# RainbowZL0/swin-unet-image-fusion

Measured on AMD Instinct MI355X. Metric: fused image-pairs/sec at 256x256, win=8, higher is better.
Workload: dtype bf16; 1 GPU; B=16/GPU 256x256 IR/visible pairs, win=8, 5-level Swin-UNet fusion forward (BASELINE configs[1]); global_batch=16, precision_mode=fast, residual_stream=fp32, hip_graph=True, steps_in_flight=3, kernel_schedule=throughput, collective=none, weights=random-init (numpy PCG64 recipe, seed 0)

## Files before the change

### swin_unet_image_fusion_amd/csrc/kernels_win48.hip

```cpp
#include "kernels_win48.h"
#include "win_frag.h"

#include <algorithm>

namespace swf {
namespace {

using namespace wf;

constexpr int W48_WAVES = 2;

template <int HID_>
struct G48 {
    static constexpr int C = 48, HID = HID_, HEADS = 8, D = 6;
    static constexpr int NT1 = HID / 32, KU = HID / 16;
    static_assert(HID % 32 == 0, "hidden tiles");
    static constexpr int F_QKV = 0;
    static constexpr int F_P = 36;
    static constexpr int F_W1 = 52;
    static constexpr int F_W2 = F_W1 + 6 * NT1;
    static constexpr int NFRAG = F_W2 + 4 * KU;
    static constexpr int V_LN1G = 0, V_LN1B = 24, V_LN2G = 48, V_LN2B = 72, V_B2 = 96, V_BQ = 120, V_BK = 152, V_B1 = 184, VHF = 288;
    static_assert(V_B1 + 16 * NT1 <= VHF, "vector block");
    static constexpr int VSTREAM = 2 * VHF + 64;
    static constexpr size_t p_vec = size_t(NFRAG) * 1024;
    static constexpr size_t p_bias = (p_vec + size_t(VSTREAM) * 4 + 15) / 16 * 16;
    static constexpr size_t p_total = p_bias + size_t(2) * 2 * 16 * 64 * 4;
    static constexpr size_t l_k = 0, l_v = 16 * 1024, l_vec = 32 * 1024, l_total = l_vec + size_t(2) * VSTREAM * 4;
    static constexpr size_t p_total16 = p_bias + size_t(15) * 16 * 64 * 4;
    static constexpr size_t l_k16 = 0, l_v16 = 32 * 1024, l_vec16 = 64 * 1024, l_total16 = l_vec16 + size_t(2) * VSTREAM * 4;
};

struct Win48Args {
    const float* in[2];
    float* out[2];
    const char* packed[2];
    const char* warm[2];
    int B, H, W, shift, cross, warm_bytes;
    int ntok[2];
};

constexpr int W48_BLOCK = 0, W48_ATTN = 1, W48_MLP = 2;

__device__ __forceinline__ void raw48(const f32x16& x0, const f32x16& x1, u32x4 (&xh)[3], u32x4 (&xl)[3]) {
    float n[24];
#pragma unroll
    for (int i = 0; i < 24; ++i) n[i] = i < 16 ? x0[i] : x1[i - 16];
    split8(n, xh[0], xl[0]);
    split8(n + 8, xh[1], xl[1]);
    split8(n + 16, xh[2], xl[2]);
}

__device__ __forceinline__ void layernorm48(const f32x16& x0, const f32x16& x1, const float* vec, int goff, int boff, u32x4 (&xh)[3], u32x4 (&xl)[3]) {
    float s = 0.f;
#pragma unroll
    for (int i = 0; i < 16; ++i) s += x0[i];
#pragma unroll
    for (int i = 0; i < 8; ++i) s += x1[i];
    const float mean = sum_halves(s) * (1.0f / 48.0f);
    float d[24], q = 0.f;
#pragma unroll
    for (int i = 0; i < 24; ++i) {
        d[i] = (i < 16 ? x0[i] : x1[i - 16]) - mean;
        q += d[i] * d[i];
    }
    const float rstd = __builtin_amdgcn_rsqf(sum_halves(q) * (1.0f / 48.0f) + 1e-5f);
    float n[24];
#pragma unroll
    for (int a = 0; a < 6; ++a) {
        const float4 g = *reinterpret_cast<const float4*>(vec + goff + 4 * a);
        const float4 b = *reinterpret_cast<const float4*>(vec + boff + 4 * a);
        n[4 * a + 0] = d[4 * a + 0] * rstd * g.x + b.x;
        n[4 * a + 1] = d[4 * a + 1] * rstd * g.y + b.y;
        n[4 * a + 2] = d[4 * a + 2] * rstd * g.z + b.z;
        n[4 * a + 3] = d[4 * a + 3] * rstd * g.w + b.w;
    }
    split8(n, xh[0], xl[0]);
    split8(n + 8, xh[1], xl[1]);
    split8(n + 16, xh[2], xl[2]);
}

__device__ __forceinline__ void attention48(const u32x4* ksrc, const u32x4* vsrc, const u32x4 (&qf)[2][2], const f32x16 (&bias)[2],
                                            bool half1, f32x16 (&o)[2]) {
    const f32x16 zero16 = {0.f, 0.f, 0.f, 0.f, 0.f, 0.f, 0.f, 0.f, 0.f, 0.f, 0.f, 0.f, 0.f, 0.f, 0.f, 0.f};
    o[0] = zero16;
    o[1] = zero16;
#pragma unroll
    for (int h = 0; h < 8; ++h) {
        const int T = h >> 2, hq = h & 3, sp = hq >> 1, sub = hq & 1;
        const u32x4 ka0 = ksrc[((0 * 2 + T) * 2 + sp) * 64], ka1 = ksrc[((1 * 2 + T) * 2 + sp) * 64];
        u32x4 qm = {0u, 0u, 0u, 0u};
        qm[2 * sub] = qf[T][sp][2 * sub];
        qm[2 * sub + 1] = qf[T][sp][2 * sub + 1];
        float mx;
        {
            f32x16 s0 = mfma_f16(ka0, qm, bias[0]);
            mx = max3f(s0[0], s0[1], s0[2]);
#pragma unroll
            for (int i = 3; i < 15; i += 2) mx = max3f(mx, s0[i], s0[i + 1]);
            mx = __builtin_fmaxf(mx, s0[15]);
        }
        {
            f32x16 s1 = mfma_f16(ka1, qm, bias[1]);
#pragma unroll
            for (int i = 0; i < 16; i += 2) mx = max3f(mx, s1[i], s1[i + 1]);
        }
        mx = max_halves(mx);
        {
            const f16 nm = (f16)(-mx);
            qm[2 * sub + 1] |= half1 ? ((unsigned)__builtin_bit_cast(unsigned short, nm) << 16) : 0u;
        }
        f32x16 t;
#pragma unroll
        for (int kt = 0; kt < 2; ++kt) {
            f32x16 sc = mfma_f16(kt ? ka1 : ka0, qm, bias[kt]);
#pragma unroll
            for (int s2 = 0; s2 < 2; ++s2) {
                float p[8];
#pragma unroll
                for (int j = 0; j < 8; ++j) p[j] = __builtin_amdgcn_exp2f(sc[8 * s2 + j]);
                const u32x4 pf = pack8_f16(p);
                const u32x4 va = vsrc[(T * 4 + 2 * kt + s2) * 64];
                t = mfma_f16(va, pf, (kt == 0 && s2 == 0) ? zero16 : t);
                __builtin_amdgcn_sched_barrier(0);
            }
        }
#pragma unroll
        for (int j = 0; j < 4; ++j) o[T][4 * hq + j] = t[4 * hq + j];
        __builtin_amdgcn_sched_barrier(0);
    }
}

template <int HID, int WS, int MODE = W48_BLOCK, bool RAW = false>
__global__ __launch_bounds__(256, W48_WAVES) void window48_kernel(Win48Args args) {
    using G = G48<HID>;
    static_assert(WS == 7 || WS == 8, "window side");
    static_assert(!RAW || MODE != W48_BLOCK, "RAW belongs to the half-block modes");
    constexpr bool ATT = MODE != W48_MLP, MLP = MODE != W48_ATTN;
    __shared__ __attribute__((aligned(16))) char smem[G::l_total];
    u32x4* kimg = reinterpret_cast<u32x4*>(smem + G::l_k);
    u32x4* vimg = reinterpret_cast<u32x4*>(smem + G::l_v);
    float* lvec = reinterpret_cast<float*>(smem + G::l_vec);

    const int tid = threadIdx.x, lane = tid & 63, wave = tid >> 6;
    const int ws = wave >> 1, qb = wave & 1, r = lane & 31, hf = lane >> 5;
    const int H = args.H, W = args.W, nwx = ATT ? W / WS : 1, nwy = ATT ? H / WS : 1, npi = nwx * nwy;
    const int nwin = ATT ? args.B * npi : (max(args.ntok[0], args.ntok[1]) + 63) / 64;
    const int sh = args.shift ? WS / 2 : 0;
    const int kvs = args.cross ? 1 - ws : ws;

    const __amdgpu_buffer_rsrc_t wrs = __builtin_amdgcn_make_buffer_rsrc(const_cast<char*>(uniform_ptr(args.packed[ws])), 0, (int)G::p_total, 0x00020000);
    const __amdgpu_buffer_rsrc_t krs = __builtin_amdgcn_make_buffer_rsrc(const_cast<char*>(uniform_ptr(args.packed[kvs])), 0, (int)G::p_total, 0x00020000);
    const int act_bytes = ATT ? args.B * H * W * 48 * 4 : args.ntok[ws] * 48 * 4;
    const __amdgpu_buffer_rsrc_t irs = __builtin_amdgcn_make_buffer_rsrc(const_cast<float*>(uniform_ptr(args.in[ws])), 0, act_bytes, 0x00020000);
    const __amdgpu_buffer_rsrc_t ors = __builtin_amdgcn_make_buffer_rsrc(uniform_ptr(args.out[ws]), 0, (MODE == W48_BLOCK || args.out[ws]) ? act_bytes : 0, 0x00020000);
    const unsigned loff = (unsigned)lane * 16u;
    auto WF = [&](int f) { return __builtin_bit_cast(u32x4, __builtin_amdgcn_raw_buffer_load_b128(wrs, loff, f * 1024, 0)); };
    auto WK = [&](int f) { return __builtin_bit_cast(u32x4, __builtin_amdgcn_raw_buffer_load_b128(krs, loff, f * 1024, 0)); };
    const float* vec = lvec + ws * G::VSTREAM + hf * G::VHF;
    const float* veck = lvec + kvs * G::VSTREAM + hf * G::VHF;
    const float* vecv = lvec + kvs * G::VSTREAM + 2 * G::VHF;
    const bool half1 = hf != 0;
    const bool col_masked = half1 != (((r >> 2) & 1) != 0);
    const f32x16 zero16 = {0.f, 0.f, 0.f, 0.f, 0.f, 0.f, 0.f, 0.f, 0.f, 0.f, 0.f, 0.f, 0.f, 0.f, 0.f, 0.f};

    for (int win = blockIdx.x; win < nwin; win += gridDim.x) {
        SWF_WF_FENCE();
        const int b = win / npi, wrem = win - b * npi;
        const int wy = wrem / nwx, wx = wrem - wy * nwx;
        const int ty = 4 * qb + (r >> 3), tx = r & 7;
        int oy = wy * WS + ty + sh, ox = wx * WS + tx + sh;
        oy = oy >= H ? oy - H : oy;
        ox = ox >= W ? ox - W : ox;
        const unsigned tokoff = [&]() -> unsigned {
            if constexpr (ATT) {
                return (WS == 8 || (ty < WS && tx < WS)) ? (unsigned)((((b * H + oy) * W + ox) * 48 + 4 * hf) * 4) : 0x80000000u;
            } else {
                const int tok = 64 * win + 32 * qb + r;
                return tok < args.ntok[ws] ? (unsigned)((tok * 48 + 4 * hf) * 4) : 0x80000000u;
            }
        }();
        auto load_rows = [&](f32x16& t0, f32x16& t1) {
#pragma unroll
            for (int a = 0; a < 6; ++a) {
                const f32x4 v = __builtin_bit_cast(f32x4, __builtin_amdgcn_raw_buffer_load_b128(irs, tokoff, 32 * a, 0));
                if (a < 4) { t0[4 * a] = v.x; t0[4 * a + 1] = v.y; t0[4 * a + 2] = v.z; t0[4 * a + 3] = v.w; }
                else { t1[4 * (a - 4)] = v.x; t1[4 * (a - 4) + 1] = v.y; t1[4 * (a - 4) + 2] = v.z; t1[4 * (a - 4) + 3] = v.w; }
            }
#pragma unroll
            for (int i = 8; i < 16; ++i) t1[i] = 0.f;
        };

        f32x16 res0, res1;
        if constexpr (ATT) {
        u32x4 qf[2][2];
        {
            u32x4 wq[2][6];
            auto req = [&](int ph, u32x4 (&dst)[6]) {
                const int m = ph >> 1, T = ph & 1;
#pragma unroll
                for (int i = 0; i < 6; ++i) dst[i] = m == 0 ? WF(G::F_QKV + ((m * 2 + T) * 3) * 2 + i) : WK(G::F_QKV + ((m * 2 + T) * 3) * 2 + i);
            };
            req(0, wq[0]);
            f32x16 x0, x1;
            load_rows(x0, x1);
            if (win == (int)blockIdx.x) {
                static_assert(G::VSTREAM % 4 == 0 && G::p_vec % 16 == 0, "vector sections move as 16-byte groups");
                    fill_vectors<G::VSTREAM / 4, 256>(lvec, args.packed[0] + G::p_vec, args.packed[1] + G::p_vec, tid);
                __syncthreads();
            }
            u32x4 xh[3], xl[3];
            if constexpr (RAW) raw48(x0, x1, xh, xl);
            else layernorm48(x0, x1, vec, G::V_LN1G, G::V_LN1B, xh, xl);
            float t[16];
#pragma unroll
            for (int ph = 0; ph < 6; ++ph) {
                const int m = ph >> 1, T = ph & 1;
                SWF_WF_FENCE();
                if (ph + 1 < 6) req(ph + 1, wq[(ph + 1) & 1]);
                SWF_WF_FENCE();
                const u32x4 (&w)[6] = wq[ph & 1];
                f32x16 acc = zero16;
                if (RAW && (m == 0 ? ws == 1 : ws == 0)) {
                    if (ph == 2 && win != (int)blockIdx.x) __syncthreads();
                } else if (m < 2) {
#pragma unroll
                    for (int s = 0; s < 3; ++s) acc = mma3(w[2 * s], w[2 * s + 1], xh[s], xl[s], acc);
                    const float* bsrc = m == 0 ? vec + G::V_BQ : veck + G::V_BK;
#pragma unroll
                    for (int g = 0; g < 4; ++g) {
                        const float4 bb = *reinterpret_cast<const float4*>(bsrc + 16 * T + 4 * g);
                        t[4 * g] = acc[4 * g] + bb.x; t[4 * g + 1] = acc[4 * g + 1] + bb.y; t[4 * g + 2] = acc[4 * g + 2] + bb.z; t[4 * g + 3] = acc[4 * g + 3] + bb.w;
                    }
                    if (m == 0) {
                        qf[T][0] = pack8_f16(t);
                        qf[T][1] = pack8_f16(t + 8);
                    } else {
                        if (T == 0 && win != (int)blockIdx.x) __syncthreads();
                        u32x4* kdst = kimg + (((kvs * 2 + qb) * 2 + T) * 2) * 64 + lane;
                        kdst[0] = pack8_f16(t);
                        kdst[64] = pack8_f16(t + 8);
                    }
                } else {
#pragma unroll
                    for (int s = 0; s < 3; ++s) acc = mma3(xh[s], xl[s], w[2 * s], w[2 * s + 1], acc);
                    const float bv = vecv[32 * T + r];
#pragma unroll
                    for (int i = 0; i < 16; ++i) t[i] = acc[i] + bv;
                    u32x4* vdst = vimg + ((kvs * 2 + T) * 4 + 2 * qb) * 64 + lane;
                    vdst[0] = pack8_f16(t);
                    vdst[64] = pack8_f16(t + 8);
                }
            }
        }
        f32x16 bias[2];
#pragma unroll
        for (int kt = 0; kt < 2; ++kt)
#pragma unroll
            for (int a = 0; a < 4; ++a) {
                const f32x4 v = __builtin_bit_cast(f32x4, __builtin_amdgcn_raw_buffer_load_b128(wrs, loff, (int)G::p_bias + ((__builtin_amdgcn_readfirstlane(qb) * 2 + kt) * 4 + a) * 1024, 0));
                bias[kt][4 * a] = v.x; bias[kt][4 * a + 1] = v.y; bias[kt][4 * a + 2] = v.z; bias[kt][4 * a + 3] = v.w;
            }
        __syncthreads();
        if (RAW && ws == 1) continue;

        f32x16 o[2];
        {
            const bool rowv = args.shift && wy == nwy - 1, colv = args.shift && wx == nwx - 1;
            const u32x4* ksrc = kimg + (ws * 8) * 64 + lane;
            const u32x4* vsrc = vimg + (ws * 8) * 64 + lane;
            if (rowv || colv) {
                const float pen0 = ((rowv && qb == 1) || (colv && col_masked)) ? -INFINITY : 0.f;
                const float pen1 = ((rowv && qb == 0) || (colv && col_masked)) ? -INFINITY : 0.f;
#pragma unroll
                for (int i = 0; i < 16; ++i) { bias[0][i] += pen0; bias[1][i] += pen1; }
            }
            attention48(ksrc, vsrc, qf, bias, half1, o);
        }

        u32x4 wpj[16];
        SWF_WF_FENCE();
        if constexpr (RAW) { res0 = zero16; res1 = zero16; }
        else load_rows(res0, res1);
#pragma unroll
        for (int i = 0; i < 16; ++i) wpj[i] = WF(G::F_P + i);
        SWF_WF_FENCE();
        {
            u32x4 oh[4], ol[4];
#pragma unroll
            for (int T = 0; T < 2; ++T) {
                float t[16];
#pragma unroll
                for (int q = 0; q < 4; ++q) {
                    float lo_, den;
                    halves(o[T][4 * q + 2], lo_, den);
                    const float inv = __builtin_amdgcn_rcpf(den);
                    t[4 * q] = o[T][4 * q] * inv; t[4 * q + 1] = o[T][4 * q + 1] * inv; t[4 * q + 2] = o[T][4 * q + 2] * inv; t[4 * q + 3] = o[T][4 * q + 3] * inv;
                }
                split8(t, oh[2 * T], ol[2 * T]);
                split8(t + 8, oh[2 * T + 1], ol[2 * T + 1]);
            }
#pragma unroll
            for (int ks = 0; ks < 4; ++ks) {
                res0 = mma3(wpj[(0 * 4 + ks) * 2], wpj[(0 * 4 + ks) * 2 + 1], oh[ks], ol[ks], res0);
                res1 = mma3(wpj[(1 * 4 + ks) * 2], wpj[(1 * 4 + ks) * 2 + 1], oh[ks], ol[ks], res1);
            }
        }

        } else {
            load_rows(res0, res1);
            if (win == (int)blockIdx.x) {
                fill_vectors<G::VSTREAM / 4, 256>(lvec, args.packed[0] + G::p_vec, args.packed[1] + G::p_vec, tid);
                __syncthreads();
            }
        }

        if constexpr (MLP) {
            u32x4 w1[2][6];
            auto req1 = [&](int tI, u32x4 (&dst)[6]) {
#pragma unroll
                for (int i = 0; i < 6; ++i) dst[i] = WF(G::F_W1 + tI * 6 + i);
            };
            u32x4 w2[2][2][2][2];
            auto req2 = [&](int tI, u32x4 (&dst)[2][2][2]) {
#pragma unroll
                for (int To = 0; To < 2; ++To)
#pragma unroll
                    for (int s2 = 0; s2 < 2; ++s2) {
                        dst[To][s2][0] = WF(G::F_W2 + (To * G::KU + 2 * tI + s2) * 2);
                        dst[To][s2][1] = WF(G::F_W2 + (To * G::KU + 2 * tI + s2) * 2 + 1);
                    }
            };
            req1(0, w1[0]);
            req2(0, w2[0]);
            u32x4 xh[3], xl[3];
            if constexpr (RAW) { raw48(res0, res1, xh, xl); res0 = zero16; res1 = zero16; }
            else layernorm48(res0, res1, vec, G::V_LN2G, G::V_LN2B, xh, xl);
#pragma unroll
            for (int tI = 0; tI < G::NT1; ++tI) {
                SWF_WF_FENCE();
                if (tI + 1 < G::NT1) { req1(tI + 1, w1[(tI + 1) & 1]); req2(tI + 1, w2[(tI + 1) & 1]); }
                SWF_WF_FENCE();
                const u32x4 (&w)[6] = w1[tI & 1];
                f32x16 acc = zero16;
#pragma unroll
                for (int s = 0; s < 3; ++s) acc = mma3(w[2 * s], w[2 * s + 1], xh[s], xl[s], acc);
                float e[16];
#pragma unroll
                for (int g = 0; g < 4; ++g) {
                    const float4 b1 = *reinterpret_cast<const float4*>(vec + G::V_B1 + 16 * tI + 4 * g);
                    const float bb[4] = {b1.x, b1.y, b1.z, b1.w};
#pragma unroll
                    for (int j = 0; j < 4; ++j) {
                        const float u = acc[4 * g + j] + bb[j];
                        const float L = __builtin_fmaf(__builtin_amdgcn_exp2f(u), kLog2e, -kLog2e);
                        e[4 * g + j] = __builtin_amdgcn_fmed3f(u, L, 0.f);
                    }
                }
#pragma unroll
                for (int s2 = 0; s2 < 2; ++s2) {
                    u32x4 hh, hl;
                    split8(e + 8 * s2, hh, hl);
                    res0 = mma3(w2[tI & 1][0][s2][0], w2[tI & 1][0][s2][1], hh, hl, res0);
                    res1 = mma3(w2[tI & 1][1][s2][0], w2[tI & 1][1][s2][1], hh, hl, res1);
                }
                __builtin_amdgcn_sched_barrier(0);
            }
#pragma unroll
            for (int a = 0; a < 6; ++a) {
                const float4 b2 = *reinterpret_cast<const float4*>(vec + G::V_B2 + 4 * a);
                if (a < 4) { res0[4 * a] += b2.x; res0[4 * a + 1] += b2.y; res0[4 * a + 2] += b2.z; res0[4 * a + 3] += b2.w; }
                else { res1[4 * (a - 4)] += b2.x; res1[4 * (a - 4) + 1] += b2.y; res1[4 * (a - 4) + 2] += b2.z; res1[4 * (a - 4) + 3] += b2.w; }
            }
        }

#pragma unroll
        for (int a = 0; a < 6; ++a) {
            const f32x4 v = a < 4 ? f32x4{res0[4 * a], res0[4 * a + 1], res0[4 * a + 2], res0[4 * a + 3]}
                                  : f32x4{res1[4 * (a - 4)], res1[4 * (a - 4) + 1], res1[4 * (a - 4) + 2], res1[4 * (a - 4) + 3]};
            __builtin_amdgcn_raw_buffer_store_b128(__builtin_bit_cast(u32x4, v), ors, tokoff, 32 * a, 0);
        }
    }

    if (args.warm[0]) {
        const int nsl = max(1, (int)gridDim.x / 8), sl = ((int)blockIdx.x / 8) % nsl;
        const int lines = (args.warm_bytes + 127) / 128;
        const int per = (lines + nsl - 1) / nsl, l0 = sl * per, l1 = min(lines, l0 + per);
        unsigned acc = 0;
        for (int s2 = 0; s2 < 2; ++s2)
            for (int l = l0 + tid; l < l1; l += 256) acc ^= *reinterpret_cast<const unsigned*>(args.warm[s2] + (size_t)l * 128);
        if (acc == 0x9e3779b9u && args.B < 0) args.out[0][0] = 0.f;
    }
}

template <int HID>
__global__ __launch_bounds__(256, 2) void window48w16_kernel(Win48Args args) {
    using G = G48<HID>;
    extern __shared__ __attribute__((aligned(16))) char smem48[];
    u32x4* kimg = reinterpret_cast<u32x4*>(smem48 + G::l_k16);
    u32x4* vimg = reinterpret_cast<u32x4*>(smem48 + G::l_v16);
    float* lvec = reinterpret_cast<float*>(smem48 + G::l_vec16);

    const int tid = threadIdx.x, lane = tid & 63, wave = tid >> 6;
    const int ws = blockIdx.y, r = lane & 31, hf = lane >> 5;
    const int H = args.H, W = args.W, nwx = W / 16, nwy = H / 16, npi = nwx * nwy;
    const int nwin = args.B * npi;
    const int sh = args.shift ? 8 : 0;
    const int src = args.cross ? 1 - ws : ws;

    static_assert(G::VSTREAM % 4 == 0 && G::p_vec % 16 == 0, "vector sections move as 16-byte groups");
                    fill_vectors<G::VSTREAM / 4, 256>(lvec, args.packed[0] + G::p_vec, args.packed[1] + G::p_vec, tid);
    const __amdgpu_buffer_rsrc_t wrs = __builtin_amdgcn_make_buffer_rsrc(const_cast<char*>(args.packed[ws]), 0, (int)G::p_total16, 0x00020000);
    const int act_bytes = args.B * H * W * 48 * 4;
    const __amdgpu_buffer_rsrc_t irs = __builtin_amdgcn_make_buffer_rsrc(const_cast<float*>(args.in[ws]), 0, act_bytes, 0x00020000);
    const __amdgpu_buffer_rsrc_t srs = __builtin_amdgcn_make_buffer_rsrc(const_cast<float*>(args.in[src]), 0, act_bytes, 0x00020000);
    const __amdgpu_buffer_rsrc_t ors = __builtin_amdgcn_make_buffer_rsrc(args.out[ws], 0, act_bytes, 0x00020000);
    const unsigned loff = (unsigned)lane * 16u;
    auto WF = [&](int f) { return __builtin_bit_cast(u32x4, __builtin_amdgcn_raw_buffer_load_b128(wrs, loff, f * 1024, 0)); };
    const float* vec = lvec + ws * G::VSTREAM + hf * G::VHF;
    const float* vecs = lvec + src * G::VSTREAM + hf * G::VHF;
    const float* vecv = lvec + ws * G::VSTREAM + 2 * G::VHF;
    const bool half1 = hf != 0;
    const f32x16 zero16 = {0.f, 0.f, 0.f, 0.f, 0.f, 0.f, 0.f, 0.f, 0.f, 0.f, 0.f, 0.f, 0.f, 0.f, 0.f, 0.f};
    __syncthreads();

    for (int win = blockIdx.x; win < nwin; win += gridDim.x) {
        SWF_WF_FENCE();
        const int b = win / npi, wrem = win - b * npi;
        const int wy = wrem / nwx, wx = wrem - wy * nwx;
        auto tokoff_of = [&](int j) {
            int oy = wy * 16 + 2 * j + (r >> 4) + sh, ox = wx * 16 + (r & 15) + sh;
            oy = oy >= H ? oy - H : oy;
            ox = ox >= W ? ox - W : ox;
            return (unsigned)((((b * H + oy) * W + ox) * 48 + 4 * hf) * 4);
        };
        auto load_rows = [&](const __amdgpu_buffer_rsrc_t& rs, unsigned tokoff, f32x16& t0, f32x16& t1) {
#pragma unroll
            for (int a = 0; a < 6; ++a) {
                const f32x4 v = __builtin_bit_cast(f32x4, __builtin_amdgcn_raw_buffer_load_b128(rs, tokoff, 32 * a, 0));
                if (a < 4) { t0[4 * a] = v.x; t0[4 * a + 1] = v.y; t0[4 * a + 2] = v.z; t0[4 * a + 3] = v.w; }
                else { t1[4 * (a - 4)] = v.x; t1[4 * (a - 4) + 1] = v.y; t1[4 * (a - 4) + 2] = v.z; t1[4 * (a - 4) + 3] = v.w; }
            }
#pragma unroll
            for (int i = 8; i < 16; ++i) t1[i] = 0.f;
        };

        u32x4 qf[2][2][2];
        {
            u32x4 xh[2][3], xl[2][3], kh[2][3], kl[2][3];
#pragma unroll
            for (int jj = 0; jj < 2; ++jj) {
                const unsigned tokoff = tokoff_of(2 * wave + jj);
                f32x16 x0, x1;
                load_rows(irs, tokoff, x0, x1);
                layernorm48(x0, x1, vec, G::V_LN1G, G::V_LN1B, xh[jj], xl[jj]);
                if (args.cross) {
                    load_rows(srs, tokoff, x0, x1);
                    layernorm48(x0, x1, vecs, G::V_LN1G, G::V_LN1B, kh[jj], kl[jj]);
                } else {
#pragma unroll
                    for (int s2 = 0; s2 < 3; ++s2) { kh[jj][s2] = xh[jj][s2]; kl[jj][s2] = xl[jj][s2]; }
                }
            }
            u32x4 wq[2][6];
            auto req = [&](int ph, u32x4 (&dst)[6]) {
#pragma unroll
                for (int i = 0; i < 6; ++i) dst[i] = WF(G::F_QKV + ph * 6 + i);
            };
            req(0, wq[0]);
#pragma unroll
            for (int ph = 0; ph < 6; ++ph) {
                const int m = ph >> 1, T = ph & 1;
                SWF_WF_FENCE();
                if (ph + 1 < 6) req(ph + 1, wq[(ph + 1) & 1]);
                SWF_WF_FENCE();
                const u32x4 (&w)[6] = wq[ph & 1];
#pragma unroll
                for (int jj = 0; jj < 2; ++jj) {
                    const int j = 2 * wave + jj;
                    f32x16 acc = zero16;
                    float t[16];
                    if (m < 2) {
#pragma unroll
                        for (int s2 = 0; s2 < 3; ++s2)
                            acc = m == 0 ? mma3(w[2 * s2], w[2 * s2 + 1], xh[jj][s2], xl[jj][s2], acc) : mma3(w[2 * s2], w[2 * s2 + 1], kh[jj][s2], kl[jj][s2], acc);
                        const float* bsrc = m == 0 ? vec + G::V_BQ : vec + G::V_BK;
#pragma unroll
                        for (int g = 0; g < 4; ++g) {
                            const float4 bb = *reinterpret_cast<const float4*>(bsrc + 16 * T + 4 * g);
                            t[4 * g] = acc[4 * g] + bb.x; t[4 * g + 1] = acc[4 * g + 1] + bb.y; t[4 * g + 2] = acc[4 * g + 2] + bb.z; t[4 * g + 3] = acc[4 * g + 3] + bb.w;
                        }
                        if (m == 0) {
                            qf[jj][T][0] = pack8_f16(t);
                            qf[jj][T][1] = pack8_f16(t + 8);
                        } else {
                            u32x4* kdst = kimg + ((j * 2 + T) * 2) * 64 + lane;
                            kdst[0] = pack8_f16(t);
                            kdst[64] = pack8_f16(t + 8);
                        }
                    } else {
#pragma unroll
                        for (int s2 = 0; s2 < 3; ++s2) acc = mma3(kh[jj][s2], kl[jj][s2], w[2 * s2], w[2 * s2 + 1], acc);
                        const float bv = vecv[32 * T + r];
#pragma unroll
                        for (int i = 0; i < 16; ++i) t[i] = acc[i] + bv;
                        u32x4* vdst = vimg + (T * 16 + 2 * j) * 64 + lane;
                        vdst[0] = pack8_f16(t);
                        vdst[64] = pack8_f16(t + 8);
                    }
                }
            }
        }
        __syncthreads();

        const bool rowv = args.shift && wy == nwy - 1, colv = args.shift && wx == nwx - 1;
#pragma unroll 1
        for (int jj = 0; jj < 2; ++jj) {
            const int j = 2 * wave + jj;
            const unsigned tokoff = tokoff_of(j);
            f32x16 o[2] = {zero16, zero16};
            float mrun[8];
#pragma unroll
            for (int h = 0; h < 8; ++h) mrun[h] = -INFINITY;
#pragma unroll 1
            for (int c = 0; c < 4; ++c) {
                if (rowv && ((j < 4) != (c < 2))) continue;
                f32x16 bias[2];
                {
                    const int d0 = __builtin_amdgcn_readfirstlane(2 * c - j + 7);
#pragma unroll
                    for (int kt = 0; kt < 2; ++kt)
#pragma unroll
                        for (int a = 0; a < 4; ++a) {
                            const f32x4 v = __builtin_bit_cast(f32x4, __builtin_amdgcn_raw_buffer_load_b128(wrs, loff, (int)G::p_bias + ((d0 + kt) * 4 + a) * 1024, 0));
                            bias[kt][4 * a] = v.x; bias[kt][4 * a + 1] = v.y; bias[kt][4 * a + 2] = v.z; bias[kt][4 * a + 3] = v.w;
                        }
                    if (colv) {
                        const bool qhi = (r & 8) != 0;
                        const float pen_lo = qhi ? -INFINITY : 0.f, pen_hi = qhi ? 0.f : -INFINITY;
#pragma unroll
                        for (int i = 0; i < 16; ++i) {
                            const float pen = ((i >> 2) & 1) ? pen_hi : pen_lo;
                            bias[0][i] += pen; bias[1][i] += pen;
                        }
                    }
                }
                const u32x4* kc = kimg + (2 * c) * 4 * 64 + lane;
#pragma unroll
                for (int h = 0; h < 8; ++h) {
                    const int T = h >> 2, hq = h & 3, sp = hq >> 1, sub = hq & 1;
                    const u32x4 ka0 = kc[((0 * 2 + T) * 2 + sp) * 64], ka1 = kc[((1 * 2 + T) * 2 + sp) * 64];
                    u32x4 qm = {0u, 0u, 0u, 0u};
                    qm[2 * sub] = qf[0][T][sp][2 * sub];
                    qm[2 * sub + 1] = qf[0][T][sp][2 * sub + 1];
                    float mx;
                    {
                        f32x16 s0 = mfma_f16(ka0, qm, bias[0]);
                        mx = max3f(s0[0], s0[1], s0[2]);
#pragma unroll
                        for (int i = 3; i < 15; i += 2) mx = max3f(mx, s0[i], s0[i + 1]);
                        mx = __builtin_fmaxf(mx, s0[15]);
                    }
                    {
                        f32x16 s1 = mfma_f16(ka1, qm, bias[1]);
#pragma unroll
                        for (int i = 0; i < 16; i += 2) mx = max3f(mx, s1[i], s1[i + 1]);
                    }
                    mx = max_halves(mx);
                    const float mold = mrun[h];
                    const f16 nm = (f16)(-__builtin_fmaxf(mold, mx));
                    const float mnew = -(float)nm;
                    const float alpha = __builtin_amdgcn_exp2f(mold - mnew);
                    mrun[h] = mnew;
                    qm[2 * sub + 1] |= half1 ? ((unsigned)__builtin_bit_cast(unsigned short, nm) << 16) : 0u;
                    f32x16 t;
#pragma unroll
                    for (int kt = 0; kt < 2; ++kt) {
                        f32x16 sc = mfma_f16(kt ? ka1 : ka0, qm, bias[kt]);
#pragma unroll
                        for (int s2 = 0; s2 < 2; ++s2) {
                            float pe[8];
#pragma unroll
                            for (int e = 0; e < 8; ++e) pe[e] = __builtin_amdgcn_exp2f(sc[8 * s2 + e]);
                            const u32x4 pf = pack8_f16(pe);
                            const u32x4 va = vimg[(T * 16 + 4 * c + 2 * kt + s2) * 64 + lane];
                            t = mfma_f16(va, pf, (kt == 0 && s2 == 0) ? zero16 : t);
                            __builtin_amdgcn_sched_barrier(0);
                        }
                    }
#pragma unroll
                    for (int e = 0; e < 4; ++e) o[T][4 * hq + e] = __builtin_fmaf(o[T][4 * hq + e], alpha, t[4 * hq + e]);
                    __builtin_amdgcn_sched_barrier(0);
                }
            }
#pragma unroll
            for (int T = 0; T < 2; ++T) { qf[0][T][0] = qf[1][T][0]; qf[0][T][1] = qf[1][T][1]; }

            f32x16 res0, res1;
            SWF_WF_FENCE();
            load_rows(irs, tokoff, res0, res1);
            {
                u32x4 oh[4], ol[4];
#pragma unroll
                for (int T = 0; T < 2; ++T) {
                    float t[16];
#pragma unroll
                    for (int q = 0; q < 4; ++q) {
                        float lo_, den;
                        halves(o[T][4 * q + 2], lo_, den);
                        const float inv = __builtin_amdgcn_rcpf(den);
                        t[4 * q] = o[T][4 * q] * inv; t[4 * q + 1] = o[T][4 * q + 1] * inv; t[4 * q + 2] = o[T][4 * q + 2] * inv; t[4 * q + 3] = o[T][4 * q + 3] * inv;
                    }
                    split8(t, oh[2 * T], ol[2 * T]);
                    split8(t + 8, oh[2 * T + 1], ol[2 * T + 1]);
                }
                SWF_WF_FENCE();
#pragma unroll
                for (int ks = 0; ks < 4; ++ks) {
                    res0 = mma3(WF(G::F_P + (0 * 4 + ks) * 2), WF(G::F_P + (0 * 4 + ks) * 2 + 1), oh[ks], ol[ks], res0);
                    res1 = mma3(WF(G::F_P + (1 * 4 + ks) * 2), WF(G::F_P + (1 * 4 + ks) * 2 + 1), oh[ks], ol[ks], res1);
                }
            }
            {
                u32x4 w1[2][6];
                auto req1 = [&](int tI, u32x4 (&dst)[6]) {
#pragma unroll
                    for (int i = 0; i < 6; ++i) dst[i] = WF(G::F_W1 + tI * 6 + i);
                };
                req1(0, w1[0]);
                u32x4 xh[3], xl[3];
                layernorm48(res0, res1, vec, G::V_LN2G, G::V_LN2B, xh, xl);
#pragma unroll
                for (int tI = 0; tI < G::NT1; ++tI) {
                    SWF_WF_FENCE();
                    u32x4 w2[2][2][2];
#pragma unroll
                    for (int To = 0; To < 2; ++To)
#pragma unroll
                        for (int s2 = 0; s2 < 2; ++s2) {
                            w2[To][s2][0] = WF(G::F_W2 + (To * G::KU + 2 * tI + s2) * 2);
                            w2[To][s2][1] = WF(G::F_W2 + (To * G::KU + 2 * tI + s2) * 2 + 1);
                        }
                    if (tI + 1 < G::NT1) req1(tI + 1, w1[(tI + 1) & 1]);
                    SWF_WF_FENCE();
                    const u32x4 (&w)[6] = w1[tI & 1];
                    f32x16 acc = zero16;
#pragma unroll
                    for (int s2 = 0; s2 < 3; ++s2) acc = mma3(w[2 * s2], w[2 * s2 + 1], xh[s2], xl[s2], acc);
                    float e[16];
#pragma unroll
                    for (int g = 0; g < 4; ++g) {
                        const float4 b1 = *reinterpret_cast<const float4*>(vec + G::V_B1 + 16 * tI + 4 * g);
                        const float bb[4] = {b1.x, b1.y, b1.z, b1.w};
#pragma unroll
                        for (int jx = 0; jx < 4; ++jx) {
                            const float u = acc[4 * g + jx] + bb[jx];
                            const float L = __builtin_fmaf(__builtin_amdgcn_exp2f(u), kLog2e, -kLog2e);
                            e[4 * g + jx] = __builtin_amdgcn_fmed3f(u, L, 0.f);
                        }
                    }
#pragma unroll
                    for (int s2 = 0; s2 < 2; ++s2) {
                        u32x4 hh, hl;
                        split8(e + 8 * s2, hh, hl);
                        res0 = mma3(w2[0][s2][0], w2[0][s2][1], hh, hl, res0);
                        res1 = mma3(w2[1][s2][0], w2[1][s2][1], hh, hl, res1);
                    }
                    __builtin_amdgcn_sched_barrier(0);
                }
#pragma unroll
                for (int a = 0; a < 6; ++a) {
                    const float4 b2 = *reinterpret_cast<const float4*>(vec + G::V_B2 + 4 * a);
                    if (a < 4) { res0[4 * a] += b2.x; res0[4 * a + 1] += b2.y; res0[4 * a + 2] += b2.z; res0[4 * a + 3] += b2.w; }
                    else { res1[4 * (a - 4)] += b2.x; res1[4 * (a - 4) + 1] += b2.y; res1[4 * (a - 4) + 2] += b2.z; res1[4 * (a - 4) + 3] += b2.w; }
                }
            }
#pragma unroll
            for (int a = 0; a < 6; ++a) {
                const f32x4 v = a < 4 ? f32x4{res0[4 * a], res0[4 * a + 1], res0[4 * a + 2], res0[4 * a + 3]}
                                      : f32x4{res1[4 * (a - 4)], res1[4 * (a - 4) + 1], res1[4 * (a - 4) + 2], res1[4 * (a - 4) + 3]};
                __builtin_amdgcn_raw_buffer_store_b128(__builtin_bit_cast(u32x4, v), ors, tokoff, 32 * a, 0);
            }
        }
        __syncthreads();
    }
}

struct Pack48Args {
    swf_block_stream_params p[2];
    char* dst[2];
    int ws;
};

__host__ __device__ constexpr int kslot(int s, int hf, int e) { return 32 * (s >> 1) + rho(8 * (s & 1) + e, hf); }

template <int HID>
__global__ __launch_bounds__(256) void pack48_kernel(Pack48Args a) {
    using G = G48<HID>;
    const int st = blockIdx.y;
    const swf_block_stream_params& p = a.p[st];
    char* dst = a.dst[st];
    const int gtid = blockIdx.x * blockDim.x + threadIdx.x, gsz = gridDim.x * blockDim.x;
    const float qscale = kLog2e / sqrtf(6.0f);
    auto bia = [](const swf_linear& l, int n) { return (l.weight && l.bias) ? l.bias[n] : 0.f; };
    auto wgt = [](const swf_linear& l, int i) { return l.weight ? l.weight[i] : 0.f; };

    for (int idx = gtid; idx < G::NFRAG * 512; idx += gsz) {
        const int f = idx >> 9, lane = (idx >> 3) & 63, e = idx & 7, r = lane & 31, hf = lane >> 5;
        float val = 0.f;
        int hl;
        if (f < G::F_P) {
            hl = f & 1;
            const int g = f >> 1, s = g % 3, T = (g / 3) & 1, m = g / 6;
            const int k = kslot(s, hf, e), head = 4 * T + (r >> 3), c = r & 7;
            const swf_linear& l = m == 0 ? p.attn.q : m == 1 ? p.attn.k : p.attn.v;
            if (c < 6 && k < 48) {
                val = wgt(l, (head * 6 + c) * 48 + k);
                if (m == 0) val *= qscale;
            }
        } else if (f < G::F_W1) {
            const int g = (f - G::F_P) >> 1, ks = g & 3, To = g >> 2;
            hl = f & 1;
            const int n = 32 * To + r, v = kslot(ks, hf, e), head = v >> 3, c = v & 7;
            if (n < 48) val = c < 6 ? wgt(p.attn.proj, n * 48 + head * 6 + c) : (v == 6 ? bia(p.attn.proj, n) : 0.f);
        } else if (f < G::F_W2) {
            const int g = (f - G::F_W1) >> 1, s = g % 3, tI = g / 3;
            hl = f & 1;
            const int k = kslot(s, hf, e), hid = 32 * tI + r;
            if (k < 48) val = wgt(p.fc1, hid * 48 + k) * kLog2e;
        } else {
            const int g = (f - G::F_W2) >> 1, u = g % G::KU, To = g / G::KU;
            hl = f & 1;
            const int n = 32 * To + r, hid = kslot(u, hf, e);
            if (n < 48) val = wgt(p.fc2, n * HID + hid) * kLn2;
        }
        const bf16 hi = (bf16)val;
        reinterpret_cast<bf16*>(dst)[idx] = hl ? (bf16)(val - (float)hi) : hi;
    }
    float* vec = reinterpret_cast<float*>(dst + G::p_vec);
    for (int i = gtid; i < G::VSTREAM; i += gsz) {
        float v = 0.f;
        if (i < 2 * G::VHF) {
            const int hf = i / G::VHF, j = i % G::VHF;
            if (j < G::V_BQ) {
                const int which = j / 24, k = j % 24;
                const int c = k < 16 ? rho(k, hf) : 32 + rho(k - 16, hf);
                v = which == 0 ? (p.ln1.gamma ? p.ln1.gamma[c] : 1.f) : which == 1 ? (p.ln1.beta ? p.ln1.beta[c] : 0.f)
                  : which == 2 ? (p.ln2.gamma ? p.ln2.gamma[c] : 1.f) : which == 3 ? (p.ln2.beta ? p.ln2.beta[c] : 0.f) : bia(p.fc2, c);
            } else if (j < G::V_B1) {
                const int isk = j >= G::V_BK, k = (j - (isk ? G::V_BK : G::V_BQ)), T = k >> 4, vch = 32 * T + rho(k & 15, hf);
                const int head = vch >> 3, c = vch & 7;
                if (c < 6) v = isk ? bia(p.attn.k, head * 6 + c) : bia(p.attn.q, head * 6 + c) * qscale;
                else if (isk && c == 7) v = 1.0f;
            } else if (j < G::V_B1 + 16 * G::NT1) {
                const int k = j - G::V_B1, hid = 32 * (k >> 4) + rho(k & 15, hf);
                v = bia(p.fc1, hid) * kLog2e;
            }
        } else {
            const int vch = i - 2 * G::VHF, head = vch >> 3, c = vch & 7;
            v = c < 6 ? bia(p.attn.v, head * 6 + c) : (c == 6 ? 1.0f : 0.f);
        }
        vec[i] = v;
    }
    float* bm = reinterpret_cast<float*>(dst + G::p_bias);
    if (!p.attn.bias_table) return;
    if (a.ws == 16) {
        for (int i = gtid; i < 15 * 16 * 64; i += gsz) {
            const int j = i & 3, lane = (i >> 2) & 63, a4 = (i >> 8) & 3, d = i >> 10;
            const int key = rho(4 * a4 + j, lane >> 5), q = lane & 31;
            const int dy = 2 * (d - 7) + (key >> 4) - (q >> 4), dx = (key & 15) - (q & 15);
            bm[i] = p.attn.bias_table[(dy + 15) * 31 + (dx + 15)] * kLog2e;
        }
        return;
    }
    for (int i = gtid; i < 2 * 2 * 16 * 64; i += gsz) {
        const int j = i & 3, lane = (i >> 2) & 63, a4 = (i >> 8) & 3, kt = (i >> 10) & 1, qb = i >> 11;
        const int key = 32 * kt + rho(4 * a4 + j, lane >> 5), q = 32 * qb + (lane & 31);
        const int ky = key >> 3, kx = key & 7, qy = q >> 3, qx = q & 7, ws = a.ws, tw = 2 * ws - 1;
        float v = 0.f;
        if (ky >= ws || kx >= ws) v = -INFINITY;
        else if (qy < ws && qx < ws) v = p.attn.bias_table[(ky - qy + ws - 1) * tw + (kx - qx + ws - 1)] * kLog2e;
        bm[i] = v;
    }
}

}

bool win48_supported(const swf_block_desc& d) {
    return d.attn.channels == 48 && d.attn.heads == 8 && d.attn.head_dim == 6 && d.attn.win_h == d.attn.win_w && (d.attn.win_h == 8 || d.attn.win_h == 7 || d.attn.win_h == 16) &&
           (d.hidden == 192 || d.hidden == 96);
}

size_t win48_packed_bytes(const swf_block_desc& d) {
    if (!win48_supported(d)) return 0;
    if (d.attn.win_h == 16) return align_up(d.hidden == 192 ? G48<192>::p_total16 : G48<96>::p_total16, 256);
    return align_up(d.hidden == 192 ? G48<192>::p_total : G48<96>::p_total, 256);
}

int pack_win48(const swf_block_desc& d, const swf_block_stream_params& px, const swf_block_stream_params& py, void* packed_x,
               void* packed_y, hipStream_t stream) {
    if (!win48_supported(d)) return fail(SWF_ERR_UNSUPPORTED, "pack_win48: shape not covered");
    Pack48Args a;
    a.p[0] = px; a.p[1] = py;
    a.dst[0] = static_cast<char*>(packed_x); a.dst[1] = static_cast<char*>(packed_y);
    a.ws = d.attn.win_h;
    if (d.hidden == 192) hipLaunchKernelGGL((pack48_kernel<192>), dim3(64, 2), dim3(256), 0, stream, a);
    else hipLaunchKernelGGL((pack48_kernel<96>), dim3(64, 2), dim3(256), 0, stream, a);
    return check_launch("pack_win48");
}

size_t win48_half_packed_bytes(int channels, int hidden) {
    if (channels != 48 || (hidden != 192 && hidden != 96)) return 0;
    return align_up(hidden == 192 ? G48<192>::p_total : G48<96>::p_total, 256);
}

int launch_win48_half(const swf_block_desc& d, int mode, int raw, const void* packed_x, const void* packed_y, const float* x_in,
                      const float* y_in, float* x_out, float* y_out, int B, int H, int W, int ntok_x, int ntok_y, hipStream_t stream) {
    const int wsd = d.attn.win_h;
    if (mode != W48_ATTN && mode != W48_MLP) return fail(SWF_ERR_UNSUPPORTED, "win48_half: mode %d", mode);
    if (d.attn.channels != 48 || (d.hidden != 192 && d.hidden != 96)) return fail(SWF_ERR_UNSUPPORTED, "win48_half: shape not covered");
    Win48Args a{};
    a.in[0] = x_in; a.in[1] = y_in; a.out[0] = x_out; a.out[1] = y_out;
    a.packed[0] = static_cast<const char*>(packed_x); a.packed[1] = static_cast<const char*>(packed_y);
    a.B = B; a.H = H; a.W = W; a.shift = d.attn.shift; a.cross = d.cross; a.ntok[0] = ntok_x; a.ntok[1] = ntok_y;
    int nwin;
    if (mode == W48_ATTN) {
        if (!win48_supported(d) || wsd == 16 || H % wsd || W % wsd) return fail(SWF_ERR_UNSUPPORTED, "win48_half: shape not covered");
        if ((int64_t)B * H * W * 48 * 4 >= (int64_t(1) << 31)) return fail(SWF_ERR_UNSUPPORTED, "win48_half: map exceeds the 2 GB buffer window");
        nwin = B * (H / wsd) * (W / wsd);
    } else {
        if ((int64_t)std::max(ntok_x, ntok_y) * 48 * 4 >= (int64_t(1) << 31) || ntok_x <= 0) return fail(SWF_ERR_UNSUPPORTED, "win48_half: token count");
        nwin = (std::max(ntok_x, ntok_y) + 63) / 64;
    }
    const dim3 grid(std::min(nwin, W48_WAVES * num_cus())), blk(256);
#define W48_LAUNCH(HID_, WS_, MODE_, RAW_) hipLaunchKernelGGL((window48_kernel<HID_, WS_, MODE_, RAW_>), grid, blk, 0, stream, a)
    if (mode == W48_ATTN) {
        if (wsd == 8) { if (raw) W48_LAUNCH(192, 8, W48_ATTN, true); else W48_LAUNCH(192, 8, W48_ATTN, false); }
        else { if (raw) W48_LAUNCH(192, 7, W48_ATTN, true); else W48_LAUNCH(192, 7, W48_ATTN, false); }
    } else if (d.hidden == 192) {
        if (raw) W48_LAUNCH(192, 8, W48_MLP, true); else W48_LAUNCH(192, 8, W48_MLP, false);
    } else {
        if (raw) W48_LAUNCH(96, 8, W48_MLP, true); else W48_LAUNCH(96, 8, W48_MLP, false);
    }
#undef W48_LAUNCH
    return check_launch("window48 (half block)");
}

int launch_win48(const swf_block_desc& d, const void* packed_x, const void* packed_y, const float* x_in, const float* y_in,
                 float* x_out, float* y_out, int B, int H, int W, hipStream_t stream, const void* next_packed_x,
                 const void* next_packed_y, size_t next_bytes) {
    const int wsd = d.attn.win_h;
    if (!win48_supported(d) || H % wsd || W % wsd) return fail(SWF_ERR_UNSUPPORTED, "win48: shape not covered");
    if ((int64_t)B * H * W * 48 * 4 >= (int64_t(1) << 31)) return fail(SWF_ERR_UNSUPPORTED, "win48: a stream of %d x %d x %d tokens exceeds the 2 GB buffer window", B, H, W);
    Win48Args a;
    a.in[0] = x_in; a.in[1] = y_in; a.out[0] = x_out; a.out[1] = y_out;
    a.packed[0] = static_cast<const char*>(packed_x); a.packed[1] = static_cast<const char*>(packed_y);
    a.warm[0] = static_cast<const char*>(next_packed_x); a.warm[1] = static_cast<const char*>(next_packed_y);
    if (!a.warm[1]) a.warm[0] = nullptr;
    a.warm_bytes = (int)(next_bytes ? next_bytes : win48_packed_bytes(d));
    a.B = B; a.H = H; a.W = W; a.shift = d.attn.shift; a.cross = d.cross;
    const int nwin = B * (H / wsd) * (W / wsd);
    if (wsd == 16) {
        const int gx = std::min(nwin, num_cus());
        if (d.hidden == 192) {
            SWF_TRY(raise_lds_limit<&window48w16_kernel<192>>((int)G48<192>::l_total16, "window48w16"));
            hipLaunchKernelGGL((window48w16_kernel<192>), dim3(gx, 2), dim3(256), G48<192>::l_total16, stream, a);
        } else {
            SWF_TRY(raise_lds_limit<&window48w16_kernel<96>>((int)G48<96>::l_total16, "window48w16"));
            hipLaunchKernelGGL((window48w16_kernel<96>), dim3(gx, 2), dim3(256), G48<96>::l_total16, stream, a);
        }
        return check_launch("window48w16");
    }
    const int grid = std::min(nwin, W48_WAVES * num_cus());
    if (wsd == 8) {
        if (d.hidden == 192) hipLaunchKernelGGL((window48_kernel<192, 8>), dim3(grid), dim3(256), 0, stream, a);
        else hipLaunchKernelGGL((window48_kernel<96, 8>), dim3(grid), dim3(256), 0, stream, a);
    } else {
        if (d.hidden == 192) hipLaunchKernelGGL((window48_kernel<192, 7>), dim3(grid), dim3(256), 0, stream, a);
        else hipLaunchKernelGGL((window48_kernel<96, 7>), dim3(grid), dim3(256), 0, stream, a);
    }
    return check_launch("window48");
}

}
```

### swin_unet_image_fusion_amd/csrc/win_frag.h

```cpp
#pragma once
#include <hip/hip_runtime.h>

namespace swf {
namespace wf {

using bf16 = __bf16;
using f16 = _Float16;
typedef bf16 bf16x8 __attribute__((ext_vector_type(8)));
typedef bf16 bf16x4 __attribute__((ext_vector_type(4)));
typedef bf16 bf16x2 __attribute__((ext_vector_type(2)));
typedef f16 f16x8 __attribute__((ext_vector_type(8)));
typedef f16 f16x4 __attribute__((ext_vector_type(4)));
typedef f16 f16x2 __attribute__((ext_vector_type(2)));
typedef float f32x16 __attribute__((ext_vector_type(16)));
typedef float f32x4 __attribute__((ext_vector_type(4)));
typedef unsigned u32x4 __attribute__((ext_vector_type(4)));

constexpr float kLog2e = 1.4426950408889634f, kLn2 = 0.6931471805599453f;

__host__ __device__ constexpr int rho(int i, int hf) { return (i & 3) + 8 * (i >> 2) + 4 * hf; }

__device__ __forceinline__ f32x16 mfma_bf16(u32x4 a, u32x4 b, f32x16 c) {
    return __builtin_amdgcn_mfma_f32_32x32x16_bf16(__builtin_bit_cast(bf16x8, a), __builtin_bit_cast(bf16x8, b), c, 0, 0, 0);
}
__device__ __forceinline__ f32x16 mfma_f16(u32x4 a, u32x4 b, f32x16 c) {
    return __builtin_amdgcn_mfma_f32_32x32x16_f16(__builtin_bit_cast(f16x8, a), __builtin_bit_cast(f16x8, b), c, 0, 0, 0);
}
__device__ __forceinline__ f32x16 mma3(u32x4 ahi, u32x4 alo, u32x4 bhi, u32x4 blo, f32x16 acc) {
    acc = mfma_bf16(alo, bhi, acc);
    acc = mfma_bf16(ahi, blo, acc);
    acc = mfma_bf16(ahi, bhi, acc);
    return acc;
}
__device__ __forceinline__ void split8(const float* v, u32x4& hi, u32x4& lo) {
#pragma unroll
    for (int p = 0; p < 4; ++p) {
        const bf16x2 h = {(bf16)v[2 * p], (bf16)v[2 * p + 1]};
        const unsigned hu = __builtin_bit_cast(unsigned, h);
        const float h0 = __builtin_bit_cast(float, hu << 16), h1 = __builtin_bit_cast(float, hu & 0xffff0000u);
        const bf16x2 l = {(bf16)(v[2 * p] - h0), (bf16)(v[2 * p + 1] - h1)};
        hi[p] = hu;
        lo[p] = __builtin_bit_cast(unsigned, l);
    }
}
__device__ __forceinline__ void split4(const float4 v, bf16x4& hi, bf16x4& lo) {
    const float f[4] = {v.x, v.y, v.z, v.w};
#pragma unroll
    for (int i = 0; i < 4; ++i) {
        hi[i] = (bf16)f[i];
        lo[i] = (bf16)(f[i] - (float)hi[i]);
    }
}
__device__ __forceinline__ u32x4 pack8_f16(const float* v) {
    u32x4 o;
#pragma unroll
    for (int p = 0; p < 4; ++p) {
        const f16x2 h = {(f16)v[2 * p], (f16)v[2 * p + 1]};
        o[p] = __builtin_bit_cast(unsigned, h);
    }
    return o;
}
__device__ __forceinline__ void halves(float v, float& a, float& b) {
    a = v;
    b = v;
    asm("s_nop 1\n\tv_permlane32_swap_b32 %0, %1" : "+v"(a), "+v"(b));
}
__device__ __forceinline__ float sum_halves(float v) { float a, b; halves(v, a, b); return a + b; }
__device__ __forceinline__ float max_halves(float v) { float a, b; halves(v, a, b); return __builtin_fmaxf(a, b); }
__device__ __forceinline__ float max3f(float a, float b, float c) { return __builtin_fmaxf(__builtin_fmaxf(a, b), c); }

__device__ __forceinline__ float elu_fast(float v) { return v > 0.f ? v : __builtin_amdgcn_exp2f(v * kLog2e) - 1.0f; }

__device__ __forceinline__ int vt_pos(int tok) {
    const int k16 = tok & 15;
    const int e = ((k16 >> 3) << 2) | (k16 & 3);
    const int h = (k16 >> 2) & 1;
    return (tok & 48) | (h << 3) | e;
}

template <typename T>
__device__ __forceinline__ T* uniform_ptr(T* p) {
    const unsigned long long v = reinterpret_cast<unsigned long long>(p);
    const unsigned lo = __builtin_amdgcn_readfirstlane((unsigned)v), hi = __builtin_amdgcn_readfirstlane((unsigned)(v >> 32));
    return reinterpret_cast<T*>(((unsigned long long)hi << 32) | lo);
}


template <int N4, int NTHREADS>
__device__ __forceinline__ void fill_vectors(float* lvec, const char* vec0, const char* vec1, int tid) {
    constexpr int PER = (2 * N4 + NTHREADS - 1) / NTHREADS;
    f32x4 tmp[PER];
#pragma unroll
    for (int k = 0; k < PER; ++k) {
        const int idx = tid + NTHREADS * k;
        if (idx < 2 * N4) tmp[k] = reinterpret_cast<const f32x4*>(idx < N4 ? vec0 : vec1)[idx < N4 ? idx : idx - N4];
    }
#pragma unroll
    for (int k = 0; k < PER; ++k) {
        const int idx = tid + NTHREADS * k;
        if (idx < 2 * N4) reinterpret_cast<f32x4*>(lvec)[idx] = tmp[k];
    }
}

}
}

#define SWF_WF_FENCE() asm volatile("" ::: "memory")
```

Measured before the change: 8502 pairs/s.

## Software-pipeline attention head score MFMAs and prefetch first MLP weight fragments

```diff
diff --git a/swin_unet_image_fusion_amd/csrc/kernels_win48.hip b/swin_unet_image_fusion_amd/csrc/kernels_win48.hip
--- a/swin_unet_image_fusion_amd/csrc/kernels_win48.hip
+++ b/swin_unet_image_fusion_amd/csrc/kernels_win48.hip
@@ -85,49 +85,73 @@
     const f32x16 zero16 = {0.f, 0.f, 0.f, 0.f, 0.f, 0.f, 0.f, 0.f, 0.f, 0.f, 0.f, 0.f, 0.f, 0.f, 0.f, 0.f};
     o[0] = zero16;
     o[1] = zero16;
-#pragma unroll
-    for (int h = 0; h < 8; ++h) {
-        const int T = h >> 2, hq = h & 3, sp = hq >> 1, sub = hq & 1;
-        const u32x4 ka0 = ksrc[((0 * 2 + T) * 2 + sp) * 64], ka1 = ksrc[((1 * 2 + T) * 2 + sp) * 64];
+    auto kfrag = [&](int j, int kt) { return ksrc[((kt * 2 + (j >> 1)) * 2 + (j & 1)) * 64]; };
+    auto qhead = [&](int h) {
+        const int T = h >> 2, sp = (h & 3) >> 1, sub = h & 1;
         u32x4 qm = {0u, 0u, 0u, 0u};
         qm[2 * sub] = qf[T][sp][2 * sub];
         qm[2 * sub + 1] = qf[T][sp][2 * sub + 1];
-        float mx;
-        {
-            f32x16 s0 = mfma_f16(ka0, qm, bias[0]);
-            mx = max3f(s0[0], s0[1], s0[2]);
-#pragma unroll
-            for (int i = 3; i < 15; i += 2) mx = max3f(mx, s0[i], s0[i + 1]);
-            mx = __builtin_fmaxf(mx, s0[15]);
-        }
-        {
-            f32x16 s1 = mfma_f16(ka1, qm, bias[1]);
-#pragma unroll
-            for (int i = 0; i < 16; i += 2) mx = max3f(mx, s1[i], s1[i + 1]);
-        }
+        return qm;
+    };
+    auto shifted = [&](int h, const f32x16& s0, const f32x16& s1) {
+        float mx = max3f(s0[0], s0[1], s0[2]);
+#pragma unroll
+        for (int i = 3; i < 15; i += 2) mx = max3f(mx, s0[i], s0[i + 1]);
+        mx = __builtin_fmaxf(mx, s0[15]);
+#pragma unroll
+        for (int i = 0; i < 16; i += 2) mx = max3f(mx, s1[i], s1[i + 1]);
         mx = max_halves(mx);
-        {
-            const f16 nm = (f16)(-mx);
-            qm[2 * sub + 1] |= half1 ? ((unsigned)__builtin_bit_cast(unsigned short, nm) << 16) : 0u;
-        }
+        const f16 nm = (f16)(-mx);
+        u32x4 qm = qhead(h);
+        qm[2 * (h & 1) + 1] |= half1 ? ((unsigned)__builtin_bit_cast(unsigned short, nm) << 16) : 0u;
+        return qm;
+    };
+    u32x4 kc0 = kfrag(0, 0), kc1 = kfrag(0, 1);
+    u32x4 kn0 = kc0, kn1 = kc1;
+    f32x16 n0, n1;
+    u32x4 qs;
+    {
+        const u32x4 q0 = qhead(0), q1 = qhead(1);
+        n0 = mfma_f16(kc0, q0, bias[0]);
+        n1 = mfma_f16(kc1, q0, bias[1]);
+        qs = shifted(0, n0, n1);
+        SWF_ISSUE_FENCE();
+        n0 = mfma_f16(kc0, q1, bias[0]);
+        n1 = mfma_f16(kc1, q1, bias[1]);
+        kn0 = kfrag(1, 0); kn1 = kfrag(1, 1);
+    }
+#pragma unroll
+    for (int h = 0; h < 8; ++h) {
+        const int T = h >> 2, hq = h & 3;
+        f32x16 sc[2];
+        sc[0] = mfma_f16(kc0, qs, bias[0]);
+        sc[1] = mfma_f16(kc1, qs, bias[1]);
+        SWF_ISSUE_FENCE();
+        if (h + 1 < 8) qs = shifted(h + 1, n0, n1);
+        if (h & 1) { kc0 = kn0; kc1 = kn1; }
+        SWF_ISSUE_FENCE();
         f32x16 t;
 #pragma unroll
         for (int kt = 0; kt < 2; ++kt) {
-            f32x16 sc = mfma_f16(kt ? ka1 : ka0, qm, bias[kt]);
 #pragma unroll
             for (int s2 = 0; s2 < 2; ++s2) {
                 float p[8];
 #pragma unroll
-                for (int j = 0; j < 8; ++j) p[j] = __builtin_amdgcn_exp2f(sc[8 * s2 + j]);
+                for (int j = 0; j < 8; ++j) p[j] = __builtin_amdgcn_exp2f(sc[kt][8 * s2 + j]);
                 const u32x4 pf = pack8_f16(p);
                 const u32x4 va = vsrc[(T * 4 + 2 * kt + s2) * 64];
                 t = mfma_f16(va, pf, (kt == 0 && s2 == 0) ? zero16 : t);
-                __builtin_amdgcn_sched_barrier(0);
-            }
-        }
+                if (kt == 0 && h + 2 < 8) {
+                    const u32x4 qn = qhead(h + 2);
+                    if (s2 == 0) n0 = mfma_f16(kn0, qn, bias[0]);
+                    else n1 = mfma_f16(kn1, qn, bias[1]);
+                }
+                SWF_ISSUE_FENCE();
+            }
+        }
+        if ((h & 1) && h + 4 < 8) { kn0 = kfrag((h >> 1) + 2, 0); kn1 = kfrag((h >> 1) + 2, 1); }
 #pragma unroll
         for (int j = 0; j < 4; ++j) o[T][4 * hq + j] = t[4 * hq + j];
-        __builtin_amdgcn_sched_barrier(0);
     }
 }
 
@@ -192,6 +216,7 @@
         };
 
         f32x16 res0, res1;
+        u32x4 w1a[6];
         if constexpr (ATT) {
         u32x4 qf[2][2];
         {
@@ -284,6 +309,10 @@
         else load_rows(res0, res1);
 #pragma unroll
         for (int i = 0; i < 16; ++i) wpj[i] = WF(G::F_P + i);
+        if constexpr (MLP) {
+#pragma unroll
+            for (int i = 0; i < 6; ++i) w1a[i] = WF(G::F_W1 + i);
+        }
         SWF_WF_FENCE();
         {
             u32x4 oh[4], ol[4];
@@ -331,7 +360,12 @@
                         dst[To][s2][1] = WF(G::F_W2 + (To * G::KU + 2 * tI + s2) * 2 + 1);
                     }
             };
-            req1(0, w1[0]);
+            if constexpr (ATT) {
+#pragma unroll
+                for (int i = 0; i < 6; ++i) w1[0][i] = w1a[i];
+            } else {
+                req1(0, w1[0]);
+            }
             req2(0, w2[0]);
             u32x4 xh[3], xl[3];
             if constexpr (RAW) { raw48(res0, res1, xh, xl); res0 = zero16; res1 = zero16; }
diff --git a/swin_unet_image_fusion_amd/csrc/win_frag.h b/swin_unet_image_fusion_amd/csrc/win_frag.h
--- a/swin_unet_image_fusion_amd/csrc/win_frag.h
+++ b/swin_unet_image_fusion_amd/csrc/win_frag.h
@@ -106,3 +106,5 @@
 }
 
 #define SWF_WF_FENCE() asm volatile("" ::: "memory")
+
+#define SWF_ISSUE_FENCE() __builtin_amdgcn_sched_barrier(0)
```

Result: no change. 8476 pairs/s (-0.3%).
